# YOUNESELBOUKNIFY/CrossModal-IMU-Video-OOD-HAR

Measured on AMD Instinct MI355X. Metric: clips/sec fwd+bwd, 16x224^2 video + 200x6 IMU, batch 32, 1/2/4/8 GPU, higher is better.
Workload: dtype bf16; 1 GPU; CrossModalModel pretrain step: VideoMAE-B 16x224^2 + IMU 6x200 PatchTST, SigLIP loss, clip 1.0, AdamW; global_batch=32, per_gpu_batch=32, parallelism=dp1

## Files before the change

crossmodal-imu-video-ood-har_amd/cmhar/_lib.py:

```python
from __future__ import annotations

import ctypes as C
import os

import torch

_HERE = os.path.dirname(os.path.abspath(__file__))
LIB_PATH = os.environ.get('CMHAR_LIB', os.path.join(_HERE, 'libcmhar.so'))

F32, BF16, F16 = 0, 1, 2
ACT_NONE, ACT_GELU, ACT_RELU, ACT_DGELU, ACT_DRELU, ACT_GELU_SAVEGRAD, ACT_MULAUX = 0, 1, 2, 3, 4, 5, 6

vp, i32, i64, f32, u64 = C.c_void_p, C.c_int, C.c_long, C.c_float, C.c_ulonglong


class Epilogue(C.Structure):
    _fields_ = [('bias', vp), ('residual', vp), ('ldr', i64), ('aux_in', vp), ('lda', i64), ('aux_out', vp),
                ('ldo', i64), ('rowadd', vp), ('rowadd_mod', i32), ('rowadd_ld', i32), ('act', i32),
                ('alpha', f32), ('beta', f32), ('pdrop', f32), ('pad_', i32), ('seed', u64), ('rowsum', vp),
                ('rowsum_beta', f32), ('colscale_lo', i32), ('colscale_hi', i32), ('colscale', f32)]


class IMULayer(C.Structure):
    _fields_ = ([(n, vp) for n in ('w_qkv', 'b_qkv', 'w_out', 'b_out', 'ln1_g', 'ln1_b', 'w_ff1', 'b_ff1', 'w_ff2',
                                   'b_ff2', 'ln2_g', 'ln2_b')] + [('eps1', f32), ('eps2', f32)] +
                [(n, vp) for n in ('qkv', 'o', 'lse', 's1', 'mu1', 'rs1', 'h1', 'fd', 's2', 'mu2', 'rs2', 'h2')])


class IMULayerGrad(C.Structure):
    _fields_ = [(n, vp) for n in ('dqkv', 'da', 'dpre', 'df2', 'gln1', 'gln2', 'dw_qkv', 'db_qkv', 'dw_out', 'db_out',
                                  'dln1_g', 'dln1_b', 'dw_ff1', 'db_ff1', 'dw_ff2', 'db_ff2', 'dln2_g', 'dln2_b')]


IMU_MAX_LAYERS = 8

_SIGS = {
    'cmhar_version': (i32, []),
    'cmhar_gemm_bf16': (i32, [i32, i32, i32, i32, i32, vp, i64, vp, i64, vp, i64, C.POINTER(Epilogue), i32, vp, vp]),
    'cmhar_gemm_bf16_phased': (i32, [i32, i32, i32, i32, i32, vp, i64, vp, i64, vp, i64, C.POINTER(Epilogue), i32, vp,
                                     vp, i32]),
    'cmhar_gemm_f16': (i32, [i32, i32, i32, i32, i32, vp, i64, vp, i64, vp, i64, C.POINTER(Epilogue), i32, vp, vp]),
    'cmhar_gemm_bf16_ws': (i64, [i32, i32, i32]),
    'cmhar_gemm_bf16_plan': (i32, [i32, i32, i32, i32, i32, i32, i32]),
    'cmhar_gemm_bf16_plan2': (i32, [i32, i32, i32, i32, i32, i32, i32, i32]),
    'cmhar_gemm_generic': (i32, [i32, i32, i32, i32, i32, i32, vp, i64, i64, i64, vp, i64, i64, i64, vp, i64, i64,
                                 C.POINTER(Epilogue), vp]),
    'cmhar_gemm_generic_splitk': (i32, [i32, i32, i32, i32, i32, i32, vp, i64, i64, vp, i64, i64, vp, i64,
                                        C.POINTER(Epilogue), vp, vp]),
    'cmhar_attention_fwd': (i32, [i32, i32, i32, i32, i32, i32, vp, i64, vp, i64, vp, i64, vp, i64, vp, f32, f32, u64,
                                  vp]),
    'cmhar_attention_fwd_opt': (i32, [i32]),
    'cmhar_attention_bwd': (i32, [i32, i32, i32, i32, i32, i32, vp, i64, vp, i64, vp, i64, vp, i64, vp, i64, vp, vp,
                                  vp, i64, vp, i64, vp, i64, f32, f32, u64, vp]),
    'cmhar_attention_bwd_prescaled': (i32, [i32, i32, i32, i32, vp, i64, vp, i64, vp, i64, vp, i64, vp, i64, vp, vp,
                                            vp, i64, vp, i64, vp, i64, f32, vp]),
    'cmhar_layernorm_fwd': (i32, [i32, i32, i32, vp, i64, vp, i64, f32, u64, vp, i64, vp, i64, vp, vp, vp, vp, f32,
                                  vp]),
    'cmhar_layernorm_bwd_ws': (i64, [i32, i32]),
    'cmhar_layernorm_bwd': (i32, [i32, i32, i32, vp, i64, vp, i64, vp, vp, vp, vp, i64, vp, i64, vp, i64, f32, u64,
                                  vp, vp, f32, vp, vp]),
    'cmhar_colsum_ws': (i64, [i32, i32]),
    'cmhar_colsum': (i32, [i32, i32, i32, vp, i64, vp, f32, f32, vp, i64, vp]),
    'cmhar_batchnorm_fwd': (i32, [i32, i32, vp, vp, vp, vp, vp, vp, vp, vp, i32, f32, f32, i32, vp, vp]),
    'cmhar_batchnorm_bwd': (i32, [i32, i32, vp, vp, vp, vp, vp, vp, vp, vp, vp, i32, i32, f32, vp]),
    'cmhar_l2normalize_fwd': (i32, [i32, i32, vp, vp, vp, f32, vp]),
    'cmhar_l2normalize_bwd': (i32, [i32, i32, vp, vp, vp, vp, f32, vp]),
    'cmhar_siglip_ws': (i64, [i32, i32]),
    'cmhar_siglip_loss': (i32, [i32, i32, i32, vp, vp, vp, vp, vp, vp, i32, i32, vp, i32, i32, vp, vp, vp, vp]),
    'cmhar_tubelet_im2col': (i32, [i32, i32, i32, i32, i32, i32, i32, i32, vp, vp, vp]),
    'cmhar_imu_embed_fwd': (i32, [i32, i32, i32, i32, i32, i32, i32, i32, vp, C.POINTER(vp), C.POINTER(vp), vp, vp,
                                  vp, vp]),
    'cmhar_imu_embed_bwd': (i32, [i32, i32, i32, i32, i32, i32, i32, i32, i32, vp, vp, vp, vp, C.POINTER(vp),
                                  C.POINTER(vp), vp]),
# ... 145 lines not shown
```

crossmodal-imu-video-ood-har_amd/cmhar/kernels.py:

```python
from __future__ import annotations

import ctypes as C
import math
import os

import torch

from . import _lib as L
from ._lib import call, ptr

class Tracer:
    def __init__(self):
        self.active = False
        self.only = None
        self.records = []

    def begin(self, name=None):
        if not self.active or (self.only is not None and name not in self.only):
            return None
        ev = torch.cuda.Event(enable_timing=True)
        ev.record()
        return ev

    def end(self, ev0, name, flops, nbytes):
# ... 252 lines not shown
        else:
            sam, sak, sbk, sbn = 1, a.stride(0), b.stride(0), 1
        s = _generic_splits(M, N, K) if splits is None else splits
        if s > 1:
            ws = workspace(s * M * N, out.device)
            call('cmhar_gemm_generic_splitk', L.dtype_code(a.dtype), L.dtype_code(out.dtype), M, N, K, s, ptr(a), sam,
                 sak, ptr(b), sbk, sbn, ptr(out), out.stride(0), C.byref(epi), ptr(ws), st)
        else:
            call('cmhar_gemm_generic', L.dtype_code(a.dtype), L.dtype_code(out.dtype), M, N, K, 1, ptr(a), sam, sak,
                 0, ptr(b), sbk, sbn, 0, ptr(out), out.stride(0), 0, C.byref(epi), st)
    return out


def linear(x, w, bias=None, *, residual=None, act=L.ACT_NONE, aux_out=None, rowadd=None, rowadd_mod=1,
           out=None, out_dtype=None, pdrop=0.0, seed=0, colscale=None):
    M, N = x.shape[0], w.shape[0]
    if out is None:
        out = torch.empty(M, N, dtype=out_dtype or x.dtype, device=x.device)
    return gemm(0, x, w, out, bias=bias, residual=residual, act=act, aux_out=aux_out, rowadd=rowadd,
                rowadd_mod=rowadd_mod, pdrop=pdrop, seed=seed, colscale=colscale)


def linear_dgrad(dy, w, *, act=L.ACT_NONE, aux_in=None, residual=None, out=None, beta=0.0, pdrop=0.0, seed=0):
    M, K = dy.shape[0], w.shape[1]
    if out is None:
        out = torch.empty(M, K, dtype=dy.dtype, device=dy.device)
    return gemm(1, dy, w, out, act=act, aux_in=aux_in, residual=residual, beta=beta, pdrop=pdrop, seed=seed)


def rowsum_supported(layout, dtype, M, N, K):
    return layout == 2 and dtype == torch.bfloat16 and M % 256 == 0 and N % 256 == 0 and K % 64 == 0


def linear_wgrad(dy, x, *, out=None, beta=0.0, bias_out=None, bias_beta=0.0, reduce_stream=None):
    N, K = dy.shape[1], x.shape[1]
    if out is None:
        out = torch.empty(N, K, dtype=torch.float32, device=dy.device)
    if bias_out is not None and not rowsum_supported(2, dy.dtype, N, K, dy.shape[0]):
        colsum(dy, bias_out, beta=bias_beta)
        bias_out = None
    return gemm(2, dy, x, out, beta=beta, rowsum=bias_out, rowsum_beta=bias_beta, reduce_stream=reduce_stream)


def colsum(x, out=None, *, alpha=1.0, beta=0.0):
    _check_2d(x, 'x')
    M, N = x.shape
    if out is None:
        out = torch.empty(N, dtype=torch.float32, device=x.device)
    n = L.lib().cmhar_colsum_ws(M, N)
    ws = workspace(n, x.device)
    call('cmhar_colsum', L.dtype_code(x.dtype), M, N, ptr(x), x.stride(0), ptr(out), alpha, beta, ptr(ws), ws.numel(),
         L.stream(x.device))
    return out


def _head_view_ok(t, B, L_, H, D, name):
    _check_2d(t, name)
    if t.shape[0] != B * L_ or t.shape[1] < H * D:
        raise ValueError(f'{name}: expected [{B * L_}, >={H * D}] got {tuple(t.shape)}')


def attention_fwd(q, k, v, out, lse, *, B, H, Lq, Lk, D, scale, pdrop=0.0, seed=0):
    for t, n, Lx in ((q, 'q', Lq), (k, 'k', Lk), (v, 'v', Lk), (out, 'o', Lq)):
        _head_view_ok(t, B, Lx, H, D, n)
    if lse.numel() < B * H * Lq or lse.dtype != torch.float32:
        raise ValueError('lse workspace')
    dt = L.dtype_code(q.dtype)
    if D not in (8, 16, 32, 64):
        raise ValueError(f'head dim {D} not supported')
    if dt in (L.BF16, L.F16) and D == 64 and pdrop == 0.0:
        for t, n in ((q, 'q'), (k, 'k'), (v, 'v'), (out, 'o')):
            _check_bf16_operand(t, n)
    ev = TRACE.begin('attn_fwd_bf16') if (dt == L.BF16 and D == 64 and pdrop == 0.0) else None
    call('cmhar_attention_fwd', dt, B, H, Lq, Lk, D, ptr(q), q.stride(0), ptr(k), k.stride(0), ptr(v), v.stride(0),
# ... 177 lines not shown
```

crossmodal-imu-video-ood-har_amd/cmhar/videomae.py:

```python
from __future__ import annotations

import json
import math
import os
import types
import warnings
from typing import List, Optional

import numpy as np
import torch
import torch.nn as nn

from . import _lib as L
from . import kernels as K
from .grads import AutogradSink
from .weights import PackedWeights


def sinusoid_table(n_position: int, d_hid: int) -> torch.Tensor:
    pos = np.arange(n_position, dtype=np.float64)[:, None]
    j = np.arange(d_hid)[None, :]
    ang = pos / np.power(10000, 2 * (j // 2) / d_hid)
    tab = np.empty_like(ang)
    tab[:, 0::2] = np.sin(ang[:, 0::2])
# ... 238 lines not shown
    st.token0 = token0_only and _token0_last_ok(m, B, dt)
    nlayer = len(m.encoder.layer)
    for layer in m.encoder.layer:
        if st.token0 and len(st.layers) == nlayer - 1:
            x, saved = _last_layer_token0_fwd(m, layer, len(st.layers), x, W, st.geom, colscale, fscale, save)
            st.layers.append(saved)
            break
        p = _layer_params(layer)
        eps = layer.layernorm_before.eps
        h1, mu1, rs1 = K.layernorm_fwd(x, p['ln1w'], p['ln1b'], eps)
        qkv = K.linear(h1, W[f'qkv{len(st.layers)}'], W.get(f'bqkv{len(st.layers)}'), colscale=colscale)
        o = torch.empty(M, Hd, dtype=dt, device=x.device)
        lse = torch.empty(B * nh * Lt, dtype=torch.float32, device=x.device)
        K.attention_fwd(qkv[:, :Hd], qkv[:, Hd:2 * Hd], qkv[:, 2 * Hd:], o, lse, B=B, H=nh, Lq=Lt, Lk=Lt, D=D,
                        scale=fscale)
        x1 = K.linear(o, W[f'o{len(st.layers)}'], p['ob'], residual=x)
        h2, mu2, rs2 = K.layernorm_fwd(x1, p['ln2w'], p['ln2b'], layer.layernorm_after.eps)
        pre = torch.empty(M, cfg.intermediate_size, dtype=dt, device=x.device) if save else None
        g = K.linear(h2, W[f'fc1_{len(st.layers)}'], p['f1b'], act=L.ACT_GELU_SAVEGRAD if save else L.ACT_GELU,
                     aux_out=pre)
        x2 = K.linear(g, W[f'fc2_{len(st.layers)}'], p['f2b'], residual=x1)
        st.layers.append((x, h1, mu1, rs1, qkv, o, lse, x1, h2, mu2, rs2, pre, g) if save else None)
        x = x2
    if m.layernorm is not None:
        xf, muf, rsf = K.layernorm_fwd(x, m.layernorm.weight, m.layernorm.bias, m.layernorm.eps)
        st.final = (x, muf, rsf) if save else None
        x = xf
    st.out = x
    return x, st


_WGRAD_STREAMS = {}
_OVERLAP_WGRAD = {'1': True, 'reduce': 'reduce'}.get(os.environ.get('CMHAR_OVERLAP_WGRAD', '0'), False)


def _wgrad_stream(dev):
    s = _WGRAD_STREAMS.get(dev)
    if s is None:
        s = _WGRAD_STREAMS[dev] = torch.cuda.Stream(dev)
    return s


def _backward_impl(m: VideoMAEBackbone, st, dx, sink, overlap_wgrad=True):
    W = m._weights()
    B, Lt, M, Hd, nh, D, scale = st.geom
    dev = dx.device

    cur = torch.cuda.current_stream(dev)
    side = _wgrad_stream(dev) if overlap_wgrad else cur
    reduce_only = overlap_wgrad == 'reduce'

    def wgrad(params, dy, x, shape, bias=None):
        out, beta = sink.dest(params, shape, dev)
        bout, bbeta = (None, 0.0)
        if bias:
            bout, bbeta = sink.dest(bias, (sum(q.numel() for q in bias),), dev)
        if side is cur or reduce_only:
            K.linear_wgrad(dy, x, out=out, beta=beta, bias_out=bout, bias_beta=bbeta,
                           reduce_stream=side if reduce_only else None)
            return
        side.wait_stream(cur)
        with torch.cuda.stream(side):
            K.linear_wgrad(dy, x, out=out, beta=beta, bias_out=bout, bias_beta=bbeta)
        dy.record_stream(side)
        x.record_stream(side)

    def done(params):
        if side is cur:
            sink.done(params)
            return
        side.wait_stream(cur)
        with torch.cuda.stream(side):
            sink.done(params)

    def ln_grads(wp, bp):
        gw, bw = sink.dest([wp], wp.shape, dev)
        gb, bb = sink.dest([bp], bp.shape, dev)
        if bw != bb:
            raise RuntimeError('LayerNorm weight/bias gradient state differs')
        return gw, gb, bw

    if m.layernorm is not None:
        x, muf, rsf = st.final
        gw, gb, beta = ln_grads(m.layernorm.weight, m.layernorm.bias)
        dx = K.layernorm_bwd(dx, x, m.layernorm.weight, muf, rsf, gw, gb, beta_acc=beta)
        sink.done([m.layernorm.weight, m.layernorm.bias])
    for li in reversed(range(len(m.encoder.layer))):
        layer = m.encoder.layer[li]
        p = _layer_params(layer)
        if isinstance(st.layers[li][0], str):
            dx = _last_layer_token0_bwd(st, li, p, W, dx, wgrad, ln_grads, sink, dev)
            done([q for q in p.values() if q is not None])
            continue
        x, h1, mu1, rs1, qkv, o, lse, x1, h2, mu2, rs2, pre, g = st.layers[li]
        st.layers[li] = None
        dpre = _dgrad(W, f'fc2_{li}', dx, act=L.ACT_MULAUX, aux_in=pre)
        wgrad([p['f2w']], dx, g, p['f2w'].shape, [p['f2b']])
        del g
        dh2 = _dgrad(W, f'fc1_{li}', dpre)
        wgrad([p['f1w']], dpre, h2, p['f1w'].shape, [p['f1b']])
        del dpre, pre
        gw2, gb2, beta = ln_grads(p['ln2w'], p['ln2b'])
        dx1 = K.layernorm_bwd(dh2, x1, p['ln2w'], mu2, rs2, gw2, gb2, dres=dx, beta_acc=beta)
        del dh2, dx
        do = _dgrad(W, f'o{li}', dx1)
        wgrad([p['ow']], dx1, o, p['ow'].shape, [p['ob']])
        dqkv = torch.empty(M, 3 * Hd, dtype=dx1.dtype, device=dev)
        attn_bwd = K.attention_bwd_prescaled if st.prescaled else K.attention_bwd
        attn_bwd(qkv[:, :Hd], qkv[:, Hd:2 * Hd], qkv[:, 2 * Hd:], o, do, lse, dqkv[:, :Hd], dqkv[:, Hd:2 * Hd],
                 dqkv[:, 2 * Hd:], B=B, H=nh, Lq=Lt, Lk=Lt, D=D, scale=scale)
        del do, o, qkv
        dh1 = _dgrad(W, f'qkv{li}', dqkv)
        wgrad([p['qw'], p['kw'], p['vw']], dqkv, h1, (3 * Hd, Hd),
              [p['qb'], p['kb'], p['vb']] if p['qb'] is not None else None)
        del dqkv
        gw1, gb1, beta = ln_grads(p['ln1w'], p['ln1b'])
        dx = K.layernorm_bwd(dh1, x, p['ln1w'], mu1, rs1, gw1, gb1, dres=dx1, beta_acc=beta)
        del dh1, dx1
        done([q for q in p.values() if q is not None])
    pe = m.embeddings.patch_embeddings.projection
    wgrad([pe.weight], dx, st.patches, (pe.weight.shape[0], pe.weight[0].numel()), [pe.bias])
    done([pe.weight, pe.bias])
    if side is not cur:
        cur.wait_stream(side)
    st.patches = None


def _last_layer_token0_bwd(st, li, p, W, dx0, wgrad, ln_grads, sink, dev):
    B, Lt, M, Hd, nh, D, scale = st.geom
    _, x, h1, mu1, rs1, q0, kv, o0, lse0, x1_0, h2_0, mu2, rs2, pre0, g0 = st.layers[li]
    st.layers[li] = None
    dpre0 = _dgrad(W, f'fc2_{li}', dx0, act=L.ACT_MULAUX, aux_in=pre0)
    wgrad([p['f2w']], dx0, g0, p['f2w'].shape, [p['f2b']])
    dh2_0 = _dgrad(W, f'fc1_{li}', dpre0)
    wgrad([p['f1w']], dpre0, h2_0, p['f1w'].shape, [p['f1b']])
    del dpre0, pre0, g0
    gw2, gb2, beta = ln_grads(p['ln2w'], p['ln2b'])
    dx1_0 = K.layernorm_bwd(dh2_0, x1_0, p['ln2w'], mu2, rs2, gw2, gb2, dres=dx0, beta_acc=beta)
    do0 = _dgrad(W, f'o{li}', dx1_0)
    wgrad([p['ow']], dx1_0, o0, p['ow'].shape, [p['ob']])
    dq0 = torch.empty(B, Hd, dtype=dx0.dtype, device=dev)
    dkv = torch.empty(M, 2 * Hd, dtype=dx0.dtype, device=dev)
    attn_bwd = K.attention_bwd_prescaled if st.prescaled else K.attention_bwd
    attn_bwd(q0, kv[:, :Hd], kv[:, Hd:], o0, do0, lse0, dq0, dkv[:, :Hd], dkv[:, Hd:], B=B, H=nh, Lq=1, Lk=Lt, D=D,
             scale=scale)
    del do0, o0
    dh1 = _dgrad(W, f'qkv{li}', dkv, rows=slice(Hd, None))
    dh1_0 = dh1.view(B, Lt, Hd)[:, 0]
# ... 78 lines not shown
```

crossmodal-imu-video-ood-har_amd/csrc/gemm_bf16.hip:

```cpp
#include "common.h"

#include <map>
#include <mutex>
#include <type_traits>

namespace {

constexpr int BM = 128, BN = 128, BK = 64, NT = 256;

__device__ __forceinline__ int kc_off(int row, int chunk) { return row * 128 + ((chunk ^ ((row >> 1) & 7)) << 4); }
__device__ __forceinline__ int mc_swz(int k) { return ((k & 3) | (((k >> 3) & 1) << 2)) << 1; }
__device__ __forceinline__ int mc_off(int k, int chunk) { return k * 256 + ((chunk ^ mc_swz(k)) << 4); }

template <bool KC>
struct Stage {
  uint4_t r[4];
  unsigned ok = 0xfu;
  template <bool BOUNDS>
  __device__ __forceinline__ void load(const bf16* __restrict__ P, long ld, int rows_total, int r0, int k0,
                                       int kend, int tid) {
    if (BOUNDS) ok = 0;
#pragma unroll
    for (int it = 0; it < 4; ++it) {
      const int c = it * NT + tid;
// ... 483 lines not shown
  for (int rr = tid >> 4; rr < BM; rr += NT / 16) {
    const int m = bm + rr;
    if (m >= M) break;
    float v[8];
    const floatx4 lo = *(const floatx4*)&T[rr * EPI_LD + cg], hi = *(const floatx4*)&T[rr * EPI_LD + cg + 4];
#pragma unroll
    for (int j = 0; j < 4; ++j) { v[j] = lo[j]; v[4 + j] = hi[j]; }
    if (raw_out) {
      float* dst = (float*)C + (long)m * ldc + n0;
      if (!BOUNDS || n0 + 8 <= N) {
        *(floatx4*)dst = lo;
        *(floatx4*)(dst + 4) = hi;
      } else {
        for (int j = 0; j < 8 && n0 + j < N; ++j) dst[j] = v[j];
      }
    } else if (!BOUNDS || n0 + 8 <= N) {
      epilogue_store8<OutT>(e, C, ldc, m, n0, v);
    } else {
      for (int j = 0; j < 8 && n0 + j < N; ++j) epilogue_store<OutT>(e, C, ldc, m, n0 + j, v[j]);
    }
  }
}

#undef As
#undef Bs

#ifndef CMHAR_NT_REDUCE_LOAD
#define CMHAR_NT_REDUCE_LOAD 1
#endif
#ifndef CMHAR_REDUCE_DEPTH
#define CMHAR_REDUCE_DEPTH 4
#endif
template <typename OutT>
__global__ void splitk_reduce_kernel(int M, int N, int splits, const float* __restrict__ P, long split_stride,
                                     OutT* __restrict__ C, long ldc, Epilogue e, int m_base = 0) {
  const long idx = (long)blockIdx.x * blockDim.x + threadIdx.x;
  if ((N & 7) == 0) {
    const long e0 = idx * 8;
    if (e0 >= (long)M * N) return;
    const int m = (int)(e0 / N) + m_base, n0 = (int)(e0 % N);
    float s[8] = {0.f, 0.f, 0.f, 0.f, 0.f, 0.f, 0.f, 0.f};
    auto ld = [&](int z, floatx4& a, floatx4& b) {
      if (CMHAR_NT_REDUCE_LOAD) {
        a = __builtin_nontemporal_load((const floatx4*)(P + z * split_stride + e0));
        b = __builtin_nontemporal_load((const floatx4*)(P + z * split_stride + e0 + 4));
      } else {
        a = *(const floatx4*)(P + z * split_stride + e0);
        b = *(const floatx4*)(P + z * split_stride + e0 + 4);
      }
    };
    auto add = [&](const floatx4& a, const floatx4& b) {
#pragma unroll
      for (int j = 0; j < 4; ++j) { s[j] += a[j]; s[4 + j] += b[j]; }
    };
    constexpr int RD = CMHAR_REDUCE_DEPTH;
    int z = 0;
    for (; z + RD - 1 < splits; z += RD) {
      floatx4 a[RD], b[RD];
#pragma unroll
      for (int u = 0; u < RD; ++u) ld(z + u, a[u], b[u]);
#pragma unroll
      for (int u = 0; u < RD; ++u) add(a[u], b[u]);
    }
    for (; z < splits; ++z) {
      floatx4 a, b;
      ld(z, a, b);
      add(a, b);
    }
    if (e.rowsum && idx < M) {
      float r = 0.f;
      for (int z = 0; z < splits; ++z) r += P[splits * split_stride + (long)z * M + idx];
      e.rowsum[idx] = e.rowsum_beta != 0.f ? r + e.rowsum_beta * e.rowsum[idx] : r;
    }
    epilogue_store8<OutT>(e, C, ldc, m, n0, s);
    return;
  }
  const long total = (long)M * N;
  if (idx >= total) return;
  const int m = (int)(idx / N), n = (int)(idx % N);
  float s = 0.f;
  for (int z = 0; z < splits; ++z) s += P[z * split_stride + idx];
  epilogue_store<OutT>(e, C, ldc, m, n, s);
}

static inline int reduce_blocks(int M, int N) {
  const long total = (long)M * N;
  return (N & 7) == 0 ? cdiv(cdiv(total, 8), 256) : cdiv(total, 256);
}

constexpr int TM2 = 256, TN2 = 256, TK2 = 64, NT2 = 512;
constexpr int EPI2_LD = 68;
constexpr int SMEM2 = 8 * 64 * EPI2_LD * 4;

__device__ __forceinline__ int mc_off512(int k, int chunk) { return k * 512 + ((chunk ^ mc_swz(k)) << 4); }

typedef __attribute__((address_space(3))) void* lds_void_ptr;

#ifndef CMHAR_GEMM8P_ASM_DMA
#define CMHAR_GEMM8P_ASM_DMA 1
#endif
__device__ __forceinline__ void dma_asm(const char* src, char* lds, int voff) {
  const unsigned long long a = (unsigned long long)src;
  uint4_t rs;
  rs[0] = __builtin_amdgcn_readfirstlane((unsigned)a);
  rs[1] = __builtin_amdgcn_readfirstlane((unsigned)(a >> 32)) & 0xffffu;
  rs[2] = 0x7fffffffu;
  rs[3] = 0x00020000u;
  const unsigned la = __builtin_amdgcn_readfirstlane((unsigned)(uintptr_t)(lds_void_ptr)lds);
  asm volatile("s_mov_b32 m0, %0\n\ts_nop 0\n\tbuffer_load_dwordx4 %1, %2, 0 offen lds" :: "s"(la), "v"(voff), "s"(rs)
               : "memory");
}


template <bool KC>
struct DmaSrc {
// ... 387 lines not shown
    base = (const char*)(P + c0);
    kstride = ld * 2;
  }
  template <bool ASM = false>
  __device__ __forceinline__ void half(int k0, char* lds, int h, int wave) const {
    if constexpr (ASM) {
#pragma unroll
      for (int t = 0; t < 2; ++t) dma_asm(base + (long)k0 * kstride, lds + h * 16384 + (2 * wave + t) * 1024, voff[h][t]);
    } else {
      const __amdgpu_buffer_rsrc_t r = __builtin_amdgcn_make_buffer_rsrc((void*)(base + (long)k0 * kstride), (short)0,
                                                                         0x7fffffff, 0x00020000);
#pragma unroll
      for (int t = 0; t < 2; ++t)
        __builtin_amdgcn_raw_ptr_buffer_load_lds(r, (lds_void_ptr)(lds + h * 16384 + (2 * wave + t) * 1024), 16,
                                                 voff[h][t], 0, 0, 0);
    }
  }
};

template <bool A_KC>
__device__ __forceinline__ bf16x8 frag8p_a(const char* lds, int r0, int kk, int lane) {
  if (A_KC) return frag256<true>(lds, r0, kk, lane);
  const char* hb = lds + (r0 >> 7) * 16384;
  const int g = lane >> 4, i = lane & 15, q = i >> 2, p = i & 3;
  const int chunk = ((r0 & 127) >> 3) + (p >> 1);
  const int k = kk * 32 + 8 * g + q;
  const short4_t lo = __builtin_amdgcn_ds_read_tr16_b64_v4i16(LDS_PTR(short4_t, hb + mc_off(k, chunk) + (p & 1) * 8));
  const short4_t hi = __builtin_amdgcn_ds_read_tr16_b64_v4i16(LDS_PTR(short4_t, hb + mc_off(k + 4, chunk) + (p & 1) * 8));
  short8_t v = {lo[0], lo[1], lo[2], lo[3], hi[0], hi[1], hi[2], hi[3]};
  return __builtin_bit_cast(bf16x8, v);
}

template <typename E, bool A_KC, bool B_KC, typename OutT, bool PFS = false, int NA = 2>
__global__ __launch_bounds__(NT2, 2) void gemm8p_kernel(int M, int N, int K, const bf16* __restrict__ A, long lda,
                                                        const bf16* __restrict__ B, long ldb, OutT* __restrict__ C,
                                                        long ldc, Epilogue e, int klen, long split_stride,
                                                        int raw_out, int ngroup) {
  static_assert(NA == 2 || NA == 3, "two or three A buffers");
  constexpr bool kAD = CMHAR_GEMM8P_ASM_DMA && (!A_KC || !B_KC);
  constexpr bool kDirect = CMHAR_EPI_DIRECT && CMHAR_GEMM8P_ABLATE == 0 && !PFS;
  constexpr bool kAblNoB = CMHAR_GEMM8P_ABLATE == 3 || CMHAR_GEMM8P_ABLATE == 5;
  constexpr bool kAblNoA = CMHAR_GEMM8P_ABLATE == 4 || CMHAR_GEMM8P_ABLATE == 5;
  __shared__ __attribute__((aligned(16))) char smem[NA == 3 ? 163840 : SMEM2];
  const int tid = threadIdx.x, lane = tid & 63;
  const int wave = __builtin_amdgcn_readfirstlane(tid >> 6);
  const int wr = wave >> 2, wc = wave & 3;
  const int tiles_n = N / TN2, tiles_m = M / TM2, ntile = tiles_m * tiles_n;
  const int rlin = xcd_remap(blockIdx.x + ntile * blockIdx.z, ntile * gridDim.z);
  const int bid = rlin % ntile, split = rlin / ntile;
  const int kbeg = split * klen, kend = min(K, kbeg + klen);
  int tm = bid / tiles_n, tn = bid % tiles_n;
  if (ngroup > 1) {
    const int cw = (tiles_n + ngroup - 1) / ngroup;
    const int gi = min(bid / (tiles_m * cw), ngroup - 1);
    const int wg = min(cw, tiles_n - gi * cw);
    const int loc = bid - gi * tiles_m * cw;
    tm = loc / wg;
    tn = gi * cw + loc % wg;
  }
  const int bm = tm * TM2, bn = tn * TN2;
  const int nk = (kend - kbeg) / TK2;
  float* const rs_slab = raw_out ? (float*)C + (long)gridDim.z * split_stride + (long)split * M : nullptr;
  C += (long)split * split_stride;
  const bool rs = !A_KC && e.rowsum != nullptr && tn == tm % tiles_n;
  const float one8[8] = {1.f, 1.f, 1.f, 1.f, 1.f, 1.f, 1.f, 1.f};
  const bf16x8 ones = pack_frag8<E>(one8);
  floatx4 accb[2] = {floatx4{0.f, 0.f, 0.f, 0.f}, floatx4{0.f, 0.f, 0.f, 0.f}};
  std::conditional_t<A_KC, DmaHalf<true>, DmaHalfM> da;
  DmaHalf<B_KC> db;
  da.init(A, lda, bm, wave, lane);
  db.init(B, ldb, bn, wave, lane);
  auto abuf = [&](int t) -> char* { return NA == 3 ? smem + (t % 3) * 32768 : smem + (t & 1) * 65536; };
  auto bbuf = [&](int t) -> char* { return NA == 3 ? smem + 98304 + (t & 1) * 32768 : smem + (t & 1) * 65536 + 32768; };

  floatx4 acc[8][4];
#pragma unroll
  for (int i = 0; i < 8; ++i)
#pragma unroll
    for (int j = 0; j < 4; ++j) acc[i][j] = floatx4{0.f, 0.f, 0.f, 0.f};
  bf16x8 af[2][4], b0[2][2], b1[2][2];

  da.template half<kAD>(kbeg, abuf(0), 0, wave);
  da.template half<kAD>(kbeg, abuf(0), 1, wave);
  db.template half<kAD>(kbeg, bbuf(0), 0, wave);
  db.template half<kAD>(kbeg, bbuf(0), 1, wave);
  da.template half<kAD>(kbeg + TK2, abuf(1), 0, wave);
  if constexpr (NA == 3) {
    da.template half<kAD>(kbeg + TK2, abuf(1), 1, wave);
    asm volatile("s_waitcnt vmcnt(4)" ::: "memory");
  } else {
    asm volatile("s_waitcnt vmcnt(2)" ::: "memory");
  }
  __builtin_amdgcn_s_barrier();
  if (wr == 1) __builtin_amdgcn_s_barrier();
  __builtin_amdgcn_sched_barrier(0);
// ... 173 lines not shown
      const floatx4 lo = *(const floatx4*)&T[rr * EPI2_LD + cg], hi = *(const floatx4*)&T[rr * EPI2_LD + cg + 4];
      if (CMHAR_GEMM8P_ABLATE == 2) {
        if (lo[0] + hi[3] == 1234.5f) ((float*)C)[tid] = lo[1];
      } else if (raw_out) {
        float* dst = (float*)C + (long)m * ldc + n0;
        *(floatx4*)dst = lo;
        *(floatx4*)(dst + 4) = hi;
      } else {
        float v[8];
#pragma unroll
        for (int j = 0; j < 4; ++j) { v[j] = lo[j]; v[4 + j] = hi[j]; }
        epilogue_store8<OutT>(e, C, ldc, m, n0, v, ps != nullptr, pre, CMHAR_EPI_BIAS_HOIST ? bh : nullptr);
      }
    };
    if constexpr (PFS) {
#pragma unroll 1
      for (int it2 = 0; it2 < 8; it2 += 2) {
        const uint4_t q0 = pw[0], q1 = pw[1];
#pragma unroll
        for (int j = 0; j + 2 < PD; ++j) pw[j] = pw[j + 2];
        if (it2 + PD < 8) {
          pw[PD - 2] = pf(it2 + PD);
          pw[PD - 1] = pf(it2 + PD + 1);
        }
        row(it2, q0);
        row(it2 + 1, q1);
      }
    } else {
#pragma unroll 2
      for (int it = 0; it < 8; ++it) row(it, pw[0]);
    }
    asm volatile("s_waitcnt lgkmcnt(0)" ::: "memory");
  }
}

__device__ __forceinline__ void swap_rows(const floatx4 (&a)[4], int p, float (&v)[8]) {
#pragma unroll
  for (int r = 0; r < 4; ++r) {
    const auto s = __builtin_amdgcn_permlane16_swap(__float_as_uint(a[2 * p][r]), __float_as_uint(a[2 * p + 1][r]),
                                                    false, false);
    v[r] = __uint_as_float(s[0]);
    v[4 + r] = __uint_as_float(s[1]);
  }
}
template <typename OutT>
__device__ __forceinline__ void epi_persist(const Epilogue& e, OutT* __restrict__ C, long ldc, int m0, int n0,
                                            int lane, const floatx4 (&acc)[8][4]) {
  typedef __attribute__((ext_vector_type(2))) float f2;
  typedef OutT __attribute__((ext_vector_type(2))) o2;
  typedef int __attribute__((ext_vector_type(4))) i4;
  int lz = lane;
  asm volatile("" : "+v"(lz));
  const int g = lz >> 4, li = lz & 15;
  const int cofs = ((g & 1) << 4) | ((g >> 1) << 3);
  const bool gp = e.act == ACT_GELU_SAVEGRAD && e.aux_out;
  const bool any_cs = e.colscale_hi > e.colscale_lo;
  f2 s2[2];
#pragma unroll
  for (int p = 0; p < 2; ++p) {
    const int col = n0 + 32 * p + cofs;
    const float sc = col >= e.colscale_lo && col < e.colscale_hi ? e.colscale : 1.f;
    s2[p] = f2{sc, sc};
  }
  OutT* const c0 = C + (long)(m0 + li) * ldc + n0 + cofs;
  auto put = [&](const i4& v, OutT* dst) __attribute__((always_inline)) {
    if (CMHAR_NT_STORE) __builtin_nontemporal_store(v, (i4*)dst);
// ... 628 lines not shown
}

extern "C" int cmhar_gemm_bf16_phased(int layout, int out_dtype, int M, int N, int K, const void* A, long lda,
                                      const void* B, long ldb, void* C, long ldc, const Epilogue* epi, int splits,
                                      void* ws, hipStream_t stream, int phases) {
  if (M <= 0 || N <= 0) return 0;
  if (phases < 1 || phases > 3) return -1;
  const bf16* a = (const bf16*)A;
  const bf16* b = (const bf16*)B;
  float* w = (float*)ws;
  Epilogue plain{};
  plain.alpha = 1.f;
  const Epilogue& e = epi ? *epi : plain;
  if ((e.colscale_lo | e.colscale_hi) & 7) return -1;
#define DISPATCH(AK, BKc)                                                                                     \
  return out_dtype == CMHAR_BF16                                                                              \
             ? launch<bf16, AK, BKc, bf16>(M, N, K, a, lda, b, ldb, (bf16*)C, ldc, e, splits, w, stream, phases)    \
             : launch<bf16, AK, BKc, float>(M, N, K, a, lda, b, ldb, (float*)C, ldc, e, splits, w, stream, phases)
  switch (layout) {
    case 0: DISPATCH(true, true);
    case 1: DISPATCH(true, false);
    case 2: DISPATCH(false, false);
    default: return -1;
  }
#undef DISPATCH
}

extern "C" int cmhar_gemm_bf16(int layout, int out_dtype, int M, int N, int K, const void* A, long lda, const void* B,
                               long ldb, void* C, long ldc, const Epilogue* epi, int splits, void* ws,
                               hipStream_t stream) {
  return cmhar_gemm_bf16_phased(layout, out_dtype, M, N, K, A, lda, B, ldb, C, ldc, epi, splits, ws, stream, 3);
}

extern "C" int cmhar_gemm_f16(int layout, int out_dtype, int M, int N, int K, const void* A, long lda, const void* B,
                              long ldb, void* C, long ldc, const Epilogue* epi, int splits, void* ws,
                              hipStream_t stream) {
  if (M <= 0 || N <= 0) return 0;
  if (layout != 0 || (out_dtype != CMHAR_F16 && out_dtype != CMHAR_F32)) return -1;
  Epilogue plain{};
  plain.alpha = 1.f;
  const Epilogue& e = epi ? *epi : plain;
  if (e.rowsum) return -3;
  if ((e.colscale_lo | e.colscale_hi) & 7) return -1;
  const bf16* a = (const bf16*)A;
  const bf16* b = (const bf16*)B;
  return out_dtype == CMHAR_F16
             ? launch<f16, true, true, f16>(M, N, K, a, lda, b, ldb, (f16*)C, ldc, e, splits, (float*)ws, stream, 3)
             : launch<f16, true, true, float>(M, N, K, a, lda, b, ldb, (float*)C, ldc, e, splits, (float*)ws, stream, 3);
}
```

include/cmhar.h:

```cpp
#ifndef CMHAR_H
#define CMHAR_H
#include <hip/hip_runtime_api.h>

#ifdef __cplusplus
extern "C" {
#endif

typedef struct CmharEpilogue {
  const float* bias;
  const void* residual;
  long ldr;
  const void* aux_in;
  long lda;
  void* aux_out;
  long ldo;
  const float* rowadd;
  int rowadd_mod;
  int rowadd_ld;
  int act;
  float alpha;
  float beta;
  float pdrop;
  int pad_;
  unsigned long long seed;
  float* rowsum;
  float rowsum_beta;
  int colscale_lo;
  int colscale_hi;
  float colscale;
} CmharEpilogue;

int cmhar_version(void);

int cmhar_gemm_bf16(int layout, int out_dtype, int M, int N, int K, const void* A, long lda, const void* B, long ldb,
                    void* C, long ldc, const CmharEpilogue* epi, int splits, void* ws, hipStream_t stream);
long cmhar_gemm_bf16_ws(int M, int N, int K);
int cmhar_gemm_bf16_plan(int layout, int M, int N, int K, int splits, int has_ws, int rowsum);
int cmhar_gemm_bf16_plan2(int layout, int M, int N, int K, int splits, int has_ws, int rowsum, int reads);
int cmhar_gemm_bf16_phased(int layout, int out_dtype, int M, int N, int K, const void* A, long lda, const void* B,
                           long ldb, void* C, long ldc, const CmharEpilogue* epi, int splits, void* ws,
                           hipStream_t stream, int phases);
int cmhar_gemm_f16(int layout, int out_dtype, int M, int N, int K, const void* A, long lda, const void* B, long ldb,
                   void* C, long ldc, const CmharEpilogue* epi, int splits, void* ws, hipStream_t stream);

int cmhar_gemm_generic(int in_dtype, int out_dtype, int M, int N, int K, int batch, const void* A, long sam,
                       long sak, long sAb, const void* B, long sbk, long sbn, long sBb, void* C, long ldc, long sCb,
                       const CmharEpilogue* epi, hipStream_t stream);
int cmhar_gemm_generic_splitk(int in_dtype, int out_dtype, int M, int N, int K, int splits, const void* A, long sam,
                              long sak, const void* B, long sbk, long sbn, void* C, long ldc,
                              const CmharEpilogue* epi, float* ws, hipStream_t stream);

int cmhar_attention_fwd(int dtype, int B, int H, int Lq, int Lk, int D, const void* Q, long ldq, const void* K,
                        long ldk, const void* V, long ldv, void* O, long ldo, float* lse, float scale, float pdrop,
                        unsigned long long seed, hipStream_t stream);
int cmhar_attention_fwd_opt(int mode);
int cmhar_attention_bwd(int dtype, int B, int H, int Lq, int Lk, int D, const void* Q, long ldq, const void* K,
                        long ldk, const void* V, long ldv, const void* O, long ldo, const void* dO, long lddo,
                        const float* lse, float* delta, void* dQ, long lddq, void* dK, long lddk, void* dV, long lddv,
                        float scale, float pdrop, unsigned long long seed, hipStream_t stream);
int cmhar_attention_bwd_prescaled(int B, int H, int Lq, int Lk, const void* Q, long ldq, const void* K, long ldk,
                                  const void* V, long ldv, const void* O, long ldo, const void* dO, long lddo,
                                  const float* lse, float* delta, void* dQ, long lddq, void* dK, long lddk, void* dV,
                                  long lddv, float scale, hipStream_t stream);

int cmhar_layernorm_fwd(int dtype, int M, int N, const void* a, long lda, const void* b, long ldb, float pdrop,
                        unsigned long long seed, void* h_out, long ldh, void* y, long ldy, const float* gamma,
                        const float* beta, float* mean, float* rstd, float eps, hipStream_t stream);
long cmhar_layernorm_bwd_ws(int M, int N);
int cmhar_layernorm_bwd(int dtype, int M, int N, const void* dy, long lddy, const void* h, long ldh,
                        const float* gamma, const float* mean, const float* rstd, const void* dres, long ldres,
                        void* dh, long lddh, void* db_out, long lddb, float pdrop, unsigned long long seed,
                        float* dgamma, float* dbeta, float beta_acc, float* ws, hipStream_t stream);

long cmhar_colsum_ws(int M, int N);
// ... 165 lines not shown
```

Baseline: 761.2 clips/sec.

## Group attention-output and QKV weight-gradient GEMMs into one split-K launch

Adds a grouped wgrad entry point that computes the out-projection and QKV weight gradients of each VideoMAE layer in a single gemm8p launch (each block runs one tile of each problem in turn), followed by a single fused split-K reduce kernel for both. The out-projection wgrad is deferred until after attention backward so it can be paired with the QKV wgrad, reducing kernel launches and tail effects on small grids. In exchange, the attention output tensor stays alive longer, the grid is sized by the larger problem so some blocks idle on the smaller one, and a __syncthreads separates the two tiles. It is enabled by default for bf16 and falls back to separate launches when the alignment checks fail.

```diff
diff --git a/crossmodal-imu-video-ood-har_amd/cmhar/_lib.py b/crossmodal-imu-video-ood-har_amd/cmhar/_lib.py
--- a/crossmodal-imu-video-ood-har_amd/cmhar/_lib.py
+++ b/crossmodal-imu-video-ood-har_amd/cmhar/_lib.py
@@ -21,6 +21,11 @@
                 ('rowsum_beta', f32), ('colscale_lo', i32), ('colscale_hi', i32), ('colscale', f32)]
 
 
+class WgradProblem(C.Structure):
+    _fields_ = [('M', i32), ('N', i32), ('splits', i32), ('A', vp), ('lda', i64), ('B', vp), ('ldb', i64), ('C', vp), ('ldc', i64),
+                ('beta', f32), ('rowsum_beta', f32), ('rowsum', vp)]
+
+
 class IMULayer(C.Structure):
     _fields_ = ([(n, vp) for n in ('w_qkv', 'b_qkv', 'w_out', 'b_out', 'ln1_g', 'ln1_b', 'w_ff1', 'b_ff1', 'w_ff2',
                                    'b_ff2', 'ln2_g', 'ln2_b')] + [('eps1', f32), ('eps2', f32)] +
@@ -39,6 +44,7 @@
     'cmhar_gemm_bf16': (i32, [i32, i32, i32, i32, i32, vp, i64, vp, i64, vp, i64, C.POINTER(Epilogue), i32, vp, vp]),
     'cmhar_gemm_bf16_phased': (i32, [i32, i32, i32, i32, i32, vp, i64, vp, i64, vp, i64, C.POINTER(Epilogue), i32, vp,
                                      vp, i32]),
+    'cmhar_gemm_bf16_wgrad_group': (i32, [i32, C.POINTER(WgradProblem), C.POINTER(WgradProblem), vp, i64, vp, i32]),
     'cmhar_gemm_f16': (i32, [i32, i32, i32, i32, i32, vp, i64, vp, i64, vp, i64, C.POINTER(Epilogue), i32, vp, vp]),
     'cmhar_gemm_bf16_ws': (i64, [i32, i32, i32]),
     'cmhar_gemm_bf16_plan': (i32, [i32, i32, i32, i32, i32, i32, i32]),
diff --git a/crossmodal-imu-video-ood-har_amd/cmhar/kernels.py b/crossmodal-imu-video-ood-har_amd/cmhar/kernels.py
--- a/crossmodal-imu-video-ood-har_amd/cmhar/kernels.py
+++ b/crossmodal-imu-video-ood-har_amd/cmhar/kernels.py
@@ -308,14 +308,83 @@
     return layout == 2 and dtype == torch.bfloat16 and M % 256 == 0 and N % 256 == 0 and K % 64 == 0
 
 
-def linear_wgrad(dy, x, *, out=None, beta=0.0, bias_out=None, bias_beta=0.0, reduce_stream=None):
+def linear_wgrad(dy, x, *, out=None, beta=0.0, bias_out=None, bias_beta=0.0, reduce_stream=None, splits=None):
     N, K = dy.shape[1], x.shape[1]
     if out is None:
         out = torch.empty(N, K, dtype=torch.float32, device=dy.device)
     if bias_out is not None and not rowsum_supported(2, dy.dtype, N, K, dy.shape[0]):
         colsum(dy, bias_out, beta=bias_beta)
         bias_out = None
-    return gemm(2, dy, x, out, beta=beta, rowsum=bias_out, rowsum_beta=bias_beta, reduce_stream=reduce_stream)
+    return gemm(2, dy, x, out, beta=beta, rowsum=bias_out, rowsum_beta=bias_beta, reduce_stream=reduce_stream,
+                splits=splits)
+
+
+def linear_wgrad_group(p0, p1, *, splits=None, reduce_stream=None):
+    (dy0, x0, out0, beta0, b0, bb0), (dy1, x1, out1, beta1, b1, bb1) = p0, p1
+    sp = tuple(splits) if isinstance(splits, (tuple, list)) else (splits, splits)
+
+    def separate():
+        linear_wgrad(dy0, x0, out=out0, beta=beta0, bias_out=b0, bias_beta=bb0, reduce_stream=reduce_stream,
+                     splits=sp[0])
+        linear_wgrad(dy1, x1, out=out1, beta=beta1, bias_out=b1, bias_beta=bb1, reduce_stream=reduce_stream,
+                     splits=sp[1])
+        return out0, out1
+
+    for t, n in ((dy0, 'dy0'), (x0, 'x0'), (out0, 'out0'), (dy1, 'dy1'), (x1, 'x1'), (out1, 'out1')):
+        _check_2d(t, n)
+    R = dy0.shape[0]
+    if not (x0.shape[0] == dy1.shape[0] == x1.shape[0] == R):
+        raise ValueError('linear_wgrad_group: the four operands must have the same number of rows')
+    dims = []
+    for dy, x, out, b in ((dy0, x0, out0, b0), (dy1, x1, out1, b1)):
+        M, N = dy.shape[1], x.shape[1]
+        if tuple(out.shape) != (M, N) or out.dtype != torch.float32:
+            raise ValueError(f'linear_wgrad_group: out must be fp32 [{M},{N}]')
+        if b is not None and (b.dtype != torch.float32 or b.numel() != M or not b.is_contiguous()):
+            raise ValueError(f'linear_wgrad_group: bias_out must be a contiguous fp32 [{M}] tensor')
+        dims.append((M, N))
+    if any(t.dtype != torch.bfloat16 for t in (dy0, x0, dy1, x1)) or R % 64 or \
+            any(M % 256 or N % 256 for M, N in dims):
+        return separate()
+    (M0, N0), (M1, N1) = dims
+    s0, s1 = (_splits_for(M, N, R) if s is None else int(s) for (M, N), s in zip(dims, sp))
+    nws = s0 * (M0 * N0 + M0) + s1 * (M1 * N1 + M1)
+    dev = out0.device
+    if reduce_stream is not None:
+        ws = torch.empty(nws, dtype=torch.float32, device=dev)
+    else:
+        ws = workspace(nws, dev)
+    prob = []
+    for (dy, x, out, beta, b, bb), s in zip((p0, p1), (s0, s1)):
+        q = L.WgradProblem()
+        q.M, q.N, q.splits = dy.shape[1], x.shape[1], s
+        q.A, q.lda, q.B, q.ldb, q.C, q.ldc = ptr(dy), dy.stride(0), ptr(x), x.stride(0), ptr(out), out.stride(0)
+        q.beta, q.rowsum, q.rowsum_beta = beta, ptr(b), bb
+        prob.append(q)
+    fn = L.lib().cmhar_gemm_bf16_wgrad_group
+    st = L.stream(dev)
+
+    def run(stream, phases):
+        rc = fn(R, C.byref(prob[0]), C.byref(prob[1]), ptr(ws), ws.numel(), stream, phases)
+        if rc not in (0, 1):
+            raise RuntimeError(f'cmhar_gemm_bf16_wgrad_group failed with code {rc}')
+        return rc == 0
+
+    name = 'gemm8p_kernel<false,false,float>'
+    ev = TRACE.begin(name) if TRACE.active else None
+    if ev is None and reduce_stream is None:
+        return (out0, out1) if run(st, 3) else separate()
+    if not run(st, 1):
+        return separate()
+    TRACE.end(ev, name, 2 * R * (M0 * N0 + M1 * N1),
+              2 * R * (M0 + N0 + M1 + N1) + 4 * (M0 * N0 + M1 * N1))
+    if reduce_stream is not None:
+        reduce_stream.wait_stream(torch.cuda.current_stream(dev))
+        run(reduce_stream.cuda_stream, 2)
+        ws.record_stream(reduce_stream)
+    else:
+        run(st, 2)
+    return out0, out1
 
 
 def colsum(x, out=None, *, alpha=1.0, beta=0.0):
diff --git a/crossmodal-imu-video-ood-har_amd/cmhar/videomae.py b/crossmodal-imu-video-ood-har_amd/cmhar/videomae.py
--- a/crossmodal-imu-video-ood-har_amd/cmhar/videomae.py
+++ b/crossmodal-imu-video-ood-har_amd/cmhar/videomae.py
@@ -294,6 +294,7 @@
 
 _WGRAD_STREAMS = {}
 _OVERLAP_WGRAD = {'1': True, 'reduce': 'reduce'}.get(os.environ.get('CMHAR_OVERLAP_WGRAD', '0'), False)
+_WGRAD_GROUP = os.environ.get('CMHAR_WGRAD_GROUP', '1') != '0'
 
 
 def _wgrad_stream(dev):
@@ -312,20 +313,31 @@
     side = _wgrad_stream(dev) if overlap_wgrad else cur
     reduce_only = overlap_wgrad == 'reduce'
 
-    def wgrad(params, dy, x, shape, bias=None):
-        out, beta = sink.dest(params, shape, dev)
-        bout, bbeta = (None, 0.0)
-        if bias:
-            bout, bbeta = sink.dest(bias, (sum(q.numel() for q in bias),), dev)
+    def wgrad(params, dy, x, shape, bias=None, group=None):
+        probs = []
+        for ps, dy_, x_, shape_, bias_ in [(params, dy, x, shape, bias)] + ([group] if group else []):
+            out, beta = sink.dest(ps, shape_, dev)
+            bout, bbeta = (None, 0.0)
+            if bias_:
+                bout, bbeta = sink.dest(bias_, (sum(q.numel() for q in bias_),), dev)
+            probs.append((dy_, x_, out, beta, bout, bbeta))
+
+        def issue(reduce_stream=None):
+            if len(probs) == 2:
+                K.linear_wgrad_group(probs[0], probs[1], reduce_stream=reduce_stream)
+                return
+            dy_, x_, out, beta, bout, bbeta = probs[0]
+            K.linear_wgrad(dy_, x_, out=out, beta=beta, bias_out=bout, bias_beta=bbeta, reduce_stream=reduce_stream)
+
         if side is cur or reduce_only:
-            K.linear_wgrad(dy, x, out=out, beta=beta, bias_out=bout, bias_beta=bbeta,
-                           reduce_stream=side if reduce_only else None)
+            issue(side if reduce_only else None)
             return
         side.wait_stream(cur)
         with torch.cuda.stream(side):
-            K.linear_wgrad(dy, x, out=out, beta=beta, bias_out=bout, bias_beta=bbeta)
-        dy.record_stream(side)
-        x.record_stream(side)
+            issue()
+        for dy_, x_, *_ in probs:
+            dy_.record_stream(side)
+            x_.record_stream(side)
 
     def done(params):
         if side is cur:
@@ -366,16 +378,22 @@
         dx1 = K.layernorm_bwd(dh2, x1, p['ln2w'], mu2, rs2, gw2, gb2, dres=dx, beta_acc=beta)
         del dh2, dx
         do = _dgrad(W, f'o{li}', dx1)
-        wgrad([p['ow']], dx1, o, p['ow'].shape, [p['ob']])
+        o_grad = ([p['ow']], dx1, o, p['ow'].shape, [p['ob']])
+        grouped = dx1.dtype == torch.bfloat16 and getattr(m, 'wgrad_group', _WGRAD_GROUP)
+        if not grouped:
+            wgrad(*o_grad)
+            o_grad = None
         dqkv = torch.empty(M, 3 * Hd, dtype=dx1.dtype, device=dev)
         attn_bwd = K.attention_bwd_prescaled if st.prescaled else K.attention_bwd
         attn_bwd(qkv[:, :Hd], qkv[:, Hd:2 * Hd], qkv[:, 2 * Hd:], o, do, lse, dqkv[:, :Hd], dqkv[:, Hd:2 * Hd],
                  dqkv[:, 2 * Hd:], B=B, H=nh, Lq=Lt, Lk=Lt, D=D, scale=scale)
-        del do, o, qkv
+        del do, qkv
+        if not grouped:
+            o = None
         dh1 = _dgrad(W, f'qkv{li}', dqkv)
         wgrad([p['qw'], p['kw'], p['vw']], dqkv, h1, (3 * Hd, Hd),
-              [p['qb'], p['kb'], p['vb']] if p['qb'] is not None else None)
-        del dqkv
+              [p['qb'], p['kb'], p['vb']] if p['qb'] is not None else None, group=o_grad)
+        del dqkv, o, o_grad
         gw1, gb1, beta = ln_grads(p['ln1w'], p['ln1b'])
         dx = K.layernorm_bwd(dh1, x, p['ln1w'], mu1, rs1, gw1, gb1, dres=dx1, beta_acc=beta)
         del dh1, dx1
diff --git a/crossmodal-imu-video-ood-har_amd/csrc/gemm_bf16.hip b/crossmodal-imu-video-ood-har_amd/csrc/gemm_bf16.hip
--- a/crossmodal-imu-video-ood-har_amd/csrc/gemm_bf16.hip
+++ b/crossmodal-imu-video-ood-har_amd/csrc/gemm_bf16.hip
@@ -539,9 +539,9 @@
 #define CMHAR_REDUCE_DEPTH 4
 #endif
 template <typename OutT>
-__global__ void splitk_reduce_kernel(int M, int N, int splits, const float* __restrict__ P, long split_stride,
-                                     OutT* __restrict__ C, long ldc, Epilogue e, int m_base = 0) {
-  const long idx = (long)blockIdx.x * blockDim.x + threadIdx.x;
+__device__ __forceinline__ void splitk_reduce_elems(long idx, int M, int N, int splits, const float* __restrict__ P,
+                                                    long split_stride, OutT* __restrict__ C, long ldc,
+                                                    const Epilogue& e, int m_base) {
   if ((N & 7) == 0) {
     const long e0 = idx * 8;
     if (e0 >= (long)M * N) return;
@@ -588,6 +588,27 @@
   float s = 0.f;
   for (int z = 0; z < splits; ++z) s += P[z * split_stride + idx];
   epilogue_store<OutT>(e, C, ldc, m, n, s);
+}
+template <typename OutT>
+__global__ void splitk_reduce_kernel(int M, int N, int splits, const float* __restrict__ P, long split_stride,
+                                     OutT* __restrict__ C, long ldc, Epilogue e, int m_base = 0) {
+  splitk_reduce_elems<OutT>((long)blockIdx.x * blockDim.x + threadIdx.x, M, N, splits, P, split_stride, C, ldc, e,
+                            m_base);
+}
+struct ReduceSide {
+  int M, N, splits;
+  const float* P;
+  float* C;
+  long ldc;
+  Epilogue e;
+};
+__global__ void splitk_reduce_group_kernel(ReduceSide r0, ReduceSide r1, int blocks0) {
+  if ((int)blockIdx.x < blocks0)
+    splitk_reduce_elems<float>((long)blockIdx.x * blockDim.x + threadIdx.x, r0.M, r0.N, r0.splits, r0.P,
+                               (long)r0.M * r0.N, r0.C, r0.ldc, r0.e, 0);
+  else
+    splitk_reduce_elems<float>((long)(blockIdx.x - blocks0) * blockDim.x + threadIdx.x, r1.M, r1.N, r1.splits, r1.P,
+                               (long)r1.M * r1.N, r1.C, r1.ldc, r1.e, 0);
 }
 
 static inline int reduce_blocks(int M, int N) {
@@ -1041,10 +1062,10 @@
 }
 
 template <typename E, bool A_KC, bool B_KC, typename OutT, bool PFS = false, int NA = 2>
-__global__ __launch_bounds__(NT2, 2) void gemm8p_kernel(int M, int N, int K, const bf16* __restrict__ A, long lda,
-                                                        const bf16* __restrict__ B, long ldb, OutT* __restrict__ C,
-                                                        long ldc, Epilogue e, int klen, long split_stride,
-                                                        int raw_out, int ngroup) {
+__device__ __forceinline__ void gemm8p_tile(int M, int N, int K, const bf16* __restrict__ A, long lda,
+                                            const bf16* __restrict__ B, long ldb, OutT* __restrict__ C, long ldc,
+                                            const Epilogue& e, int klen, long split_stride, int raw_out, int ngroup,
+                                            int bid, int split, int nsplit) {
   static_assert(NA == 2 || NA == 3, "two or three A buffers");
   constexpr bool kAD = CMHAR_GEMM8P_ASM_DMA && (!A_KC || !B_KC);
   constexpr bool kDirect = CMHAR_EPI_DIRECT && CMHAR_GEMM8P_ABLATE == 0 && !PFS;
@@ -1054,9 +1075,7 @@
   const int tid = threadIdx.x, lane = tid & 63;
   const int wave = __builtin_amdgcn_readfirstlane(tid >> 6);
   const int wr = wave >> 2, wc = wave & 3;
-  const int tiles_n = N / TN2, tiles_m = M / TM2, ntile = tiles_m * tiles_n;
-  const int rlin = xcd_remap(blockIdx.x + ntile * blockIdx.z, ntile * gridDim.z);
-  const int bid = rlin % ntile, split = rlin / ntile;
+  const int tiles_n = N / TN2, tiles_m = M / TM2;
   const int kbeg = split * klen, kend = min(K, kbeg + klen);
   int tm = bid / tiles_n, tn = bid % tiles_n;
   if (ngroup > 1) {
@@ -1069,7 +1088,7 @@
   }
   const int bm = tm * TM2, bn = tn * TN2;
   const int nk = (kend - kbeg) / TK2;
-  float* const rs_slab = raw_out ? (float*)C + (long)gridDim.z * split_stride + (long)split * M : nullptr;
+  float* const rs_slab = raw_out ? (float*)C + (long)nsplit * split_stride + (long)split * M : nullptr;
   C += (long)split * split_stride;
   const bool rs = !A_KC && e.rowsum != nullptr && tn == tm % tiles_n;
   const float one8[8] = {1.f, 1.f, 1.f, 1.f, 1.f, 1.f, 1.f, 1.f};
@@ -1309,6 +1328,48 @@
     }
     asm volatile("s_waitcnt lgkmcnt(0)" ::: "memory");
   }
+}
+
+template <typename E, bool A_KC, bool B_KC, typename OutT, bool PFS = false, int NA = 2>
+__global__ __launch_bounds__(NT2, 2) void gemm8p_kernel(int M, int N, int K, const bf16* __restrict__ A, long lda,
+                                                        const bf16* __restrict__ B, long ldb, OutT* __restrict__ C,
+                                                        long ldc, Epilogue e, int klen, long split_stride,
+                                                        int raw_out, int ngroup) {
+  const int ntile = (M / TM2) * (N / TN2);
+  const int rlin = xcd_remap(blockIdx.x + ntile * blockIdx.z, ntile * gridDim.z);
+  gemm8p_tile<E, A_KC, B_KC, OutT, PFS, NA>(M, N, K, A, lda, B, ldb, C, ldc, e, klen, split_stride, raw_out, ngroup,
+                                            rlin % ntile, rlin / ntile, gridDim.z);
+}
+
+struct WgradSide {
+  const bf16* A;
+  long lda;
+  const bf16* B;
+  long ldb;
+  float* ws;
+  int M, N;
+  int klen, nsplit;
+  int rowsum;
+};
+struct WgradGroup {
+  WgradSide p[2];
+};
+template <typename E, int NA>
+__device__ __forceinline__ void wgrad_group_block(const WgradSide& s, int K) {
+  const int ntile = (s.M / TM2) * (s.N / TN2);
+  if ((int)blockIdx.x >= ntile * s.nsplit) return;
+  const int rlin = xcd_remap(blockIdx.x, ntile * s.nsplit);
+  Epilogue e{};
+  e.alpha = 1.f;
+  e.rowsum = s.rowsum ? s.ws : nullptr;
+  gemm8p_tile<E, false, false, float, false, NA>(s.M, s.N, K, s.A, s.lda, s.B, s.ldb, s.ws, s.N, e, s.klen,
+                                                 (long)s.M * s.N, 1, 1, rlin % ntile, rlin / ntile, s.nsplit);
+}
+template <typename E, int NA>
+__global__ __launch_bounds__(NT2, 2) void gemm8p_wgrad_group_kernel(WgradGroup g, int K) {
+  wgrad_group_block<E, NA>(g.p[0], K);
+  __syncthreads();
+  wgrad_group_block<E, NA>(g.p[1], K);
 }
 
 __device__ __forceinline__ void swap_rows(const floatx4 (&a)[4], int p, float (&v)[8]) {
@@ -2003,6 +2064,54 @@
   return cmhar_gemm_bf16_phased(layout, out_dtype, M, N, K, A, lda, B, ldb, C, ldc, epi, splits, ws, stream, 3);
 }
 
+extern "C" int cmhar_gemm_bf16_wgrad_group(int K, const CmharWgradProblem* p0, const CmharWgradProblem* p1, void* ws,
+                                           long ws_floats, hipStream_t stream, int phases) {
+  if (phases < 1 || phases > 3) return -1;
+  if (!p0 || !p1 || !ws || K <= 0 || K % TK2 || !use_8p_wgrad()) return 1;
+  const CmharWgradProblem* q[2] = {p0, p1};
+  int klen[2], nsplit[2];
+  long nws[2];
+  for (int i = 0; i < 2; ++i) {
+    const CmharWgradProblem* p = q[i];
+    if (p->M <= 0 || p->N <= 0 || p->M % TM2 || p->N % TN2 || p->splits < 2) return 1;
+    if (!p->A || !p->B || !p->C || p->lda < p->M || p->ldb < p->N || p->ldc < p->N) return 1;
+    if (((uintptr_t)p->A | (uintptr_t)p->B | (uintptr_t)p->C) & 15) return 1;
+    if (p->lda % 8 || p->ldb % 8 || p->ldc % 8 || ((uintptr_t)p->rowsum & 3)) return 1;
+    klen[i] = cdiv(cdiv(K, p->splits), TK2) * TK2;
+    nsplit[i] = cdiv(K, klen[i]);
+    if (nsplit[i] < 2 || klen[i] < 2 * TK2 || K - (nsplit[i] - 1) * klen[i] < 2 * TK2) return 1;
+    nws[i] = (long)nsplit[i] * ((long)p->M * p->N + p->M);
+  }
+  if (ws_floats < nws[0] + nws[1] || ((uintptr_t)ws & 15)) return 1;
+  float* const w[2] = {(float*)ws, (float*)ws + nws[0]};
+  if (phases & 1) {
+    WgradGroup g;
+    for (int i = 0; i < 2; ++i)
+      g.p[i] = WgradSide{(const bf16*)q[i]->A, q[i]->lda, (const bf16*)q[i]->B, q[i]->ldb, w[i], q[i]->M, q[i]->N,
+                         klen[i], nsplit[i], q[i]->rowsum != nullptr};
+    const int grid = std::max((p0->M / TM2) * (p0->N / TN2) * nsplit[0], (p1->M / TM2) * (p1->N / TN2) * nsplit[1]);
+    if (gemm8p_na(false) == 3)
+      gemm8p_wgrad_group_kernel<bf16, 3><<<grid, NT2, 0, stream>>>(g, K);
+    else
+      gemm8p_wgrad_group_kernel<bf16, 2><<<grid, NT2, 0, stream>>>(g, K);
+    CMHAR_CHECK_LAUNCH();
+  }
+  if (phases & 2) {
+    ReduceSide r[2];
+    for (int i = 0; i < 2; ++i) {
+      r[i] = ReduceSide{q[i]->M, q[i]->N, nsplit[i], w[i], q[i]->C, q[i]->ldc, Epilogue{}};
+      r[i].e.alpha = 1.f;
+      r[i].e.beta = q[i]->beta;
+      r[i].e.rowsum = q[i]->rowsum;
+      r[i].e.rowsum_beta = q[i]->rowsum_beta;
+    }
+    const int b0 = reduce_blocks(p0->M, p0->N), b1 = reduce_blocks(p1->M, p1->N);
+    splitk_reduce_group_kernel<<<b0 + b1, 256, 0, stream>>>(r[0], r[1], b0);
+    CMHAR_CHECK_LAUNCH();
+  }
+  return 0;
+}
+
 extern "C" int cmhar_gemm_f16(int layout, int out_dtype, int M, int N, int K, const void* A, long lda, const void* B,
                               long ldb, void* C, long ldc, const Epilogue* epi, int splits, void* ws,
                               hipStream_t stream) {
diff --git a/include/cmhar.h b/include/cmhar.h
--- a/include/cmhar.h
+++ b/include/cmhar.h
@@ -40,6 +40,21 @@
 int cmhar_gemm_bf16_phased(int layout, int out_dtype, int M, int N, int K, const void* A, long lda, const void* B,
                            long ldb, void* C, long ldc, const CmharEpilogue* epi, int splits, void* ws,
                            hipStream_t stream, int phases);
+typedef struct CmharWgradProblem {
+  int M, N;
+  int splits;
+  const void* A;
+  long lda;
+  const void* B;
+  long ldb;
+  float* C;
+  long ldc;
+  float beta;
+  float rowsum_beta;
+  float* rowsum;
+} CmharWgradProblem;
+int cmhar_gemm_bf16_wgrad_group(int K, const CmharWgradProblem* p0, const CmharWgradProblem* p1, void* ws,
+                                long ws_floats, hipStream_t stream, int phases);
 int cmhar_gemm_f16(int layout, int out_dtype, int M, int N, int K, const void* A, long lda, const void* B, long ldb,
                    void* C, long ldc, const CmharEpilogue* epi, int splits, void* ws, hipStream_t stream);
 
```

Result: no change. 764.4 clips/sec (median of 4 runs) (+0.4%).
